# thebasilisk/mirror-maze

Measured on AMD Instinct MI355X. Metric: Mrays/sec + ms/frame at 1920x1080, 8 spp, 8 bounces; 1/2/4/8-GPU scaling, higher is better.
Workload: dtype f32

## Files before the change

### mirror-maze_amd/csrc/grid_build.cpp

```cpp
#include <algorithm>
#include <cmath>
#include <cstdint>
#include <cstring>
#include <string>
#include <vector>

#include "grid_build.h"
#include "mm_types.h"

namespace mm {

size_t build_compact_rects(const mm_rect* rects, uint32_t n_rects, const uint32_t* idx, std::vector<uint32_t>& out,
                           size_t* n_slow);

namespace {

void rect_box(const mm_rect& r, double lo[3], double hi[3]) {
    for (int a = 0; a < 3; ++a) {
        const double c[4] = {r.o[a], (double)r.o[a] + r.v[a], (double)r.o[a] + r.u[a],
                             (double)r.o[a] + r.v[a] + r.u[a]};
        lo[a] = *std::min_element(c, c + 4);
        hi[a] = *std::max_element(c, c + 4);
    }
}
// ... 251 lines not shown
    }
    g.n_list = (uint32_t)ext.size();
    g.off_list = align16(8u * (uint32_t)total);
    g.off_recs = align16(g.off_list + 2u * g.n_list);
    g.off_box = align16(g.off_recs + 32u * n_rects);
    g.bytes = align16(g.off_box + 24u * n_rects);
    g.image.assign(g.bytes, 0);
    std::memcpy(&g.image[0], words.data(), 8 * (size_t)total);
    if (!ext.empty()) std::memcpy(&g.image[g.off_list], ext.data(), 2 * ext.size());
    return true;
}

}

bool build_grid(const mm_rect* rects, uint32_t n_rects, const mm_node* nodes, uint32_t n_nodes,
                const uint32_t* idx, size_t index_budget, GridHost& g, std::string& why, bool merge_axes,
                double cell_scale, bool wide) {
    if (n_rects == 0 || n_rects > 65535) { why = "rect count outside 1..65535"; return false; }
    std::vector<uint32_t> ident(n_rects), recs;
    for (uint32_t k = 0; k < n_rects; ++k) ident[k] = k;
    size_t n_slow = 0;
    build_compact_rects(rects, n_rects, ident.data(), recs, &n_slow);
    double smin[3] = {INFINITY, INFINITY, INFINITY}, smax[3] = {-INFINITY, -INFINITY, -INFINITY}, C = 1.0;
    std::vector<double> ext2;
    for (uint32_t k = 0; k < n_rects; ++k) {
        double lo[3], hi[3];
        rect_box(rects[k], lo, hi);
        double e[3];
        for (int a = 0; a < 3; ++a) {
            if (!std::isfinite(lo[a]) || !std::isfinite(hi[a])) { why = "non-finite rect"; return false; }
            smin[a] = std::min(smin[a], lo[a]);
            smax[a] = std::max(smax[a], hi[a]);
            C = std::max(C, std::max(std::fabs(lo[a]), std::fabs(hi[a])));
            e[a] = hi[a] - lo[a];
        }
        std::sort(e, e + 3);
        if (e[1] > 0.0) ext2.push_back(e[1]);
    }
    if (ext2.empty()) { why = "no rect with area"; return false; }
    std::nth_element(ext2.begin(), ext2.begin() + ext2.size() / 2, ext2.end());
    std::vector<uint32_t> grecs;
    const uint32_t n_slow_g = grid_records(recs, n_rects, grecs);
    std::vector<uint32_t> cls;
    std::vector<uint32_t> cls_of(n_rects, 0);
    bool classes_ok = n_slow_g == 0;
    auto y_first = [&](uint32_t k) { return ((grecs[8 * (size_t)k + 7] >> 20) & 3u) == 2u; };
    for (uint32_t k = 0; k < n_rects && classes_ok; ++k) {
        const uint32_t* g8 = &grecs[8 * (size_t)k + 3];
        uint32_t t[4] = {g8[0], g8[1], g8[2], g8[3]};
        if (y_first(k)) { std::swap(t[0], t[2]); std::swap(t[1], t[3]); }
        uint32_t c = 0;
        while (c < cls.size() / 4 && !std::equal(t, t + 4, &cls[4 * c])) ++c;
        if (c == cls.size() / 4) {
            if (c == kMaxClasses) { classes_ok = false; break; }
            cls.insert(cls.end(), t, t + 4);
        }
        cls_of[k] = c;
    }
    auto maze_form = [&](const GridHost& gg) {
        if (gg.n[1] != 1 || !classes_ok || n_rects > 8191u) return false;
        for (uint32_t k = 0; k < n_rects; ++k) {
            const uint32_t meta = grecs[8 * (size_t)k + 7];
            const bool global = std::find(gg.glob, gg.glob + gg.n_glob, k) != gg.glob + gg.n_glob;
            if (!global && (meta >> 30) == 0u && ((meta >> 20) & 3u) == 1u) return false;
        }
        return true;
    };
    auto compact_layout = [&](GridHost& gg) {
        gg.off_class = gg.off_data = align16(gg.off_list + 2u * gg.n_list);
        gg.off_recs = gg.off_class + kGridClassBytes;
        gg.off_box = align16(gg.off_recs + 16u * n_rects);
        gg.bytes = align16(gg.off_box + 24u * n_rects);
    };
    double s = ext2[ext2.size() / 2] * cell_scale;
    for (int attempt = 0; attempt < 24; ++attempt, s *= 1.25) {
        if (wide && build_lists(rects, n_rects, recs, smin, smax, C, s, true, merge_axes, g, why)) {
            const bool mf = maze_form(g);
            if (mf) compact_layout(g);
            bool whole = false;
            for (size_t c = 0; mf && c < (size_t)g.n[0] * g.n[1] * g.n[2]; ++c)
                whole |= (g.image[8 * c + 7] & 0x80u) != 0;
            if (g.bytes <= index_budget && !whole) break;
        }
        if (build_lists(rects, n_rects, recs, smin, smax, C, s, false, merge_axes, g, why) &&
            g.off_recs <= index_budget)
            break;
        if (attempt == 23) { why = "no grid index fits the LDS budget"; return false; }
    }
    g.n_slow = n_slow_g;
    g.flat_ok = maze_form(g);
    if (g.wide && g.flat_ok) {
        for (size_t c = 0; c < (size_t)g.n[0] * g.n[1] * g.n[2]; ++c) {
            uint64_t w;
            std::memcpy(&w, &g.image[8 * c], 8);
            const uint64_t xf = (w >> 25) & 0xFFFull;
            w = (w & ~(0xFFFull << 37)) | (xf << 37);
            std::memcpy(&g.image[8 * c], &w, 8);
        }
    }
    g.slab = false;
    if (g.n_glob == 2) {
        const uint32_t m0 = grecs[8 * (size_t)g.glob[0] + 7], m1 = grecs[8 * (size_t)g.glob[1] + 7];
        const bool y_fast = (m0 >> 30) == 0u && (m1 >> 30) == 0u && ((m0 >> 20) & 3u) == 1u && ((m1 >> 20) & 3u) == 1u;
        float y0, y1;
        std::memcpy(&y0, &grecs[8 * (size_t)g.glob[0]], 4);
        std::memcpy(&y1, &grecs[8 * (size_t)g.glob[1]], 4);
        if (y_fast && y0 != y1 && std::isfinite(y0) && std::isfinite(y1)) {
            if (y1 < y0) { std::swap(g.glob[0], g.glob[1]); std::swap(y0, y1); }
            g.slab = true;
            g.slab_y[0] = y0;
            g.slab_y[1] = y1;
        }
    }
    if (g.flat_ok) {
        g.n_class = (uint32_t)cls.size() / 4;
        compact_layout(g);
        g.image.resize(g.bytes);
        std::memset(&g.image[g.off_recs], 0, g.bytes - g.off_recs);
        for (uint32_t k = 0; k < n_rects; ++k) {
            const uint32_t* w = &grecs[8 * (size_t)k];
            const uint32_t meta = (w[7] & (3u << 20)) | (cls_of[k] << 4) | (w[7] & (3u << 30));
            const uint32_t r[4] = {w[0], y_first(k) ? w[2] : w[1], y_first(k) ? w[1] : w[2], meta};
            std::memcpy(&g.image[g.off_recs + 16u * k], r, 16);
        }
        std::memcpy(&g.image[g.off_class], cls.data(), 4 * cls.size());
        for (uint32_t i = 0; i < g.n_list; ++i) {
            uint16_t e;
            std::memcpy(&e, &g.image[g.off_list + 2u * i], 2);
            e = (uint16_t)(8u * e);
            std::memcpy(&g.image[g.off_list + 2u * i], &e, 2);
        }
    } else {
        g.off_class = 0;
        g.off_data = g.off_recs;
        g.off_box = align16(g.off_recs + 32u * n_rects);
        g.bytes = align16(g.off_box + 24u * n_rects);
        g.image.resize(g.bytes);
        std::memcpy(&g.image[g.off_recs], grecs.data(), 32u * (size_t)n_rects);
    }
    std::vector<float> box(6 * (size_t)n_rects);
    for (uint32_t k = 0; k < n_rects; ++k) {
        const float e[6] = {INFINITY, -INFINITY, INFINITY, -INFINITY, INFINITY, -INFINITY};
        std::memcpy(&box[6 * (size_t)k], e, sizeof e);
    }
    for (uint32_t i = 0; i < n_nodes; ++i) {
        const mm_node& nd = nodes[i];
        if (nd.count == 0) continue;
        for (uint32_t j = 0; j < nd.count; ++j) {
            const uint32_t k = idx[nd.left_first + j];
            const float b[6] = {nd.mn[0], nd.mx[0], nd.mn[1], nd.mx[1], nd.mn[2], nd.mx[2]};
            std::memcpy(&box[6 * (size_t)k], b, sizeof b);
        }
    }
    std::memcpy(&g.image[g.off_box], box.data(), 24u * (size_t)n_rects);
    return true;
}

}
```

### mirror-maze_amd/csrc/grid_build.h

```cpp
#pragma once

#include <cstddef>
#include <cstdint>
#include <string>
#include <vector>

#include "mm_types.h"

namespace mm {

constexpr uint32_t kMaxClasses = 64;
constexpr uint32_t kGridClassBytes = 16 * kMaxClasses;

struct GridHost {
    float mn[3], mx[3], cell[3], inv[3];
    int n[3];
    uint32_t n_glob = 0;
    uint32_t glob[4] = {0, 0, 0, 0};
    uint32_t off_list = 0, off_recs = 0, off_box = 0, bytes = 0;
    uint32_t n_list = 0;
    uint32_t n_slow = 0;
    bool wide = true;
    bool flat_ok = false;
    bool slab = false;
    float slab_y[2] = {0.0f, 0.0f};
    uint32_t off_class = 0, n_class = 0;
    uint32_t off_data = 0;
    std::vector<uint8_t> image;
};

bool build_grid(const mm_rect* rects, uint32_t n_rects, const mm_node* nodes, uint32_t n_nodes,
                const uint32_t* idx, size_t index_budget, GridHost& g, std::string& why, bool merge_axes = true,
                double cell_scale = 1.0, bool wide = true);

}
```

### mirror-maze_amd/csrc/mm_device.h

```cpp
#pragma once

#include <hip/hip_runtime.h>
#include <stdint.h>

#include "grid_build.h"
#include "mm_types.h"
#include "mm_variants.h"

namespace mm {

constexpr float kBig = 1e30f;
constexpr int kStackMax = 50;

constexpr uint32_t kLaneStatRecord = 49152;
#ifdef MM_LANE_STATS
__device__ __forceinline__ uint32_t* lane_stat_words() {
    __shared__ uint32_t words[2 * kLpCount];
    return words;
}
__device__ __forceinline__ void lane_stat(int ph) {
    const uint64_t m = __ballot(1);
    if (__lane_id() == (uint32_t)(__ffsll((unsigned long long)m) - 1)) {
        atomicAdd(lane_stat_words() + 2 * ph, 1u);
        atomicAdd(lane_stat_words() + 2 * ph + 1, (uint32_t)__popcll(m));
    }
}
#define MM_LANE_STAT(ph) ::mm::lane_stat(::mm::ph)
#else
#define MM_LANE_STAT(ph) ((void)0)
#endif

__host__ __device__ constexpr bool grid_form(int f) { return f >= kFormGrid && f <= kFormGridWideSlow + kFormGridFlat; }
__host__ __device__ constexpr bool grid_flat(int f) { return f > kFormGridWideSlow; }
__host__ __device__ constexpr int grid_base(int f) { return grid_flat(f) ? f - kFormGridFlat : f; }
__host__ __device__ constexpr bool grid_slow(int f) { return grid_base(f) == kFormGridSlow || grid_base(f) == kFormGridWideSlow; }
__host__ __device__ constexpr bool grid_wide(int f) { return grid_base(f) >= kFormGridWide; }

struct DevGrid {
    float mn[3], mx[3];
    float cell[3], inv[3];
    int n[3];
    uint32_t n_glob;
    uint32_t glob[4];
    const void* cells;
    const uint16_t* list;
    const uint4* recs;
    const float2* box;
    const uint4* image;
    uint32_t off_list, off_recs, off_box, bytes;
    const float4* cls;
    uint32_t off_class;
    uint32_t off_data;
    uint32_t slab;
    float slab_y[2];
    int nm1[3];
    float nf[3];
};
inline DevGrid dev_grid(const GridHost& gh, const uint8_t* image_dev) {
    DevGrid dg{};
    for (int a = 0; a < 3; ++a) {
        dg.mn[a] = gh.mn[a]; dg.mx[a] = gh.mx[a]; dg.cell[a] = gh.cell[a]; dg.inv[a] = gh.inv[a];
        dg.n[a] = gh.n[a];
        dg.nm1[a] = gh.n[a] - 1;
        dg.nf[a] = (float)gh.n[a];
    }
    dg.n_glob = gh.n_glob;
    dg.slab = gh.slab ? 1u : 0u;
    dg.slab_y[0] = gh.slab_y[0];
    dg.slab_y[1] = gh.slab_y[1];
    for (int i = 0; i < 4; ++i) dg.glob[i] = gh.glob[i];
    dg.cells = image_dev;
    dg.list = reinterpret_cast<const uint16_t*>(image_dev + gh.off_list);
    dg.recs = reinterpret_cast<const uint4*>(image_dev + gh.off_recs);
    dg.box = reinterpret_cast<const float2*>(image_dev + gh.off_box);
    dg.image = reinterpret_cast<const uint4*>(image_dev);
    dg.off_list = gh.off_list; dg.off_recs = gh.off_recs; dg.off_box = gh.off_box; dg.bytes = gh.bytes;
    dg.off_class = gh.off_class;
    dg.off_data = gh.off_data;
    dg.cls = gh.off_class ? reinterpret_cast<const float4*>(image_dev + gh.off_class) : nullptr;
    return dg;
}

struct DevScene {
    const float4* nodes;
    const float4* nodes_ref;
    const float4* geo;
    const float4* shade;
    const uint32_t* idx;
    uint32_t n_nodes;
    uint32_t n_rects;
    uint32_t root_packed;
    uint32_t fast_ok;
    const uint2* recs;
    DevGrid grid;
};

struct F3 { float x, y, z; };
__device__ __forceinline__ F3 f3(float x, float y, float z) { return F3{x, y, z}; }
__device__ __forceinline__ F3 operator+(F3 a, F3 b) { return F3{a.x + b.x, a.y + b.y, a.z + b.z}; }
__device__ __forceinline__ F3 operator-(F3 a, F3 b) { return F3{a.x - b.x, a.y - b.y, a.z - b.z}; }
__device__ __forceinline__ F3 operator*(F3 a, F3 b) { return F3{a.x * b.x, a.y * b.y, a.z * b.z}; }
__device__ __forceinline__ F3 operator*(float s, F3 a) { return F3{s * a.x, s * a.y, s * a.z}; }
__device__ __forceinline__ float dot3(F3 a, F3 b) {
    float s = a.x * b.x;
    s = s + a.y * b.y;
    return s + a.z * b.z;
}
__device__ __forceinline__ float rsq_ieee(float x) { return 1.0f / sqrtf(x); }
__device__ __forceinline__ float rsq(float x) {
    if (x >= 0x1p-40f && x <= 0x1p40f) {
        float s = __builtin_amdgcn_sqrtf(x);
        const float sd = __uint_as_float(__float_as_uint(s) - 1u), su = __uint_as_float(__float_as_uint(s) + 1u);
        const float vd = __builtin_fmaf(-sd, s, x), vu = __builtin_fmaf(-su, s, x);
        s = vd <= 0.0f ? sd : s;
        s = vu > 0.0f ? su : s;
        const float y = __builtin_amdgcn_rcpf(s);
        const float e = __builtin_fmaf(-s, y, 1.0f);
        return __builtin_fmaf(e, y, y);
    }
    return rsq_ieee(x);
}
__device__ __forceinline__ F3 normalize3(F3 v) { return rsq(dot3(v, v)) * v; }
__device__ __forceinline__ F3 cross3(F3 v, F3 u) {
    return F3{u.z * v.y - u.y * v.z, u.x * v.z - u.z * v.x, u.y * v.x - u.x * v.y};
}
__device__ __forceinline__ F3 xyz(float4 a) { return F3{a.x, a.y, a.z}; }

__device__ __forceinline__ float rand_pm1(uint32_t& state) {
    uint32_t s = state * 747796405u + 291336453u;
    state = s;
    uint32_t r = ((s >> ((s >> 28) + 4u)) ^ s) * 277803737u;
    r = (r >> 22) ^ r;
    return __builtin_fmaf((float)r, 0x1p-31f, -1.0f);
}

__device__ __forceinline__ uint32_t cvt_u32_sat(float f) {
    if (!(f > 0.0f)) return 0u;
    if (f >= 4294967296.0f) return 0xFFFFFFFFu;
    return (uint32_t)f;
}

__device__ __forceinline__ uint32_t seed_reference(uint32_t tx, uint32_t ty, uint32_t time) {
    const float n = 128.0f / 255.0f;
    float s = n + (float)(tx * 15823u);
    s = s + n;
    s = s + (float)(ty * 9737333u);
    s = s + (float)time;
    return cvt_u32_sat(s);
}

__device__ __forceinline__ uint32_t pcg_hash(uint32_t v) {
    uint32_t s = v * 747796405u + 2891336453u;
    uint32_t w = ((s >> ((s >> 28) + 4u)) ^ s) * 277803737u;
    return (w >> 22) ^ w;
}
__device__ __forceinline__ uint32_t seed_tile(uint32_t pixel, uint32_t sample, uint32_t frame) {
    return pcg_hash(pcg_hash(pcg_hash(frame) ^ pixel) + sample);
}

__device__ __forceinline__ F3 primary_dir(const mm_uniform& u, uint32_t px, uint32_t py) {
    const float fx = (float)px, fy = (float)py;
    const float vx = u.cam.viewport[0], vy = u.cam.viewport[1];
    F3 p = F3{(vx * fx) / u.view_w - vx * 0.5f, (vy * fy) / u.view_h - vy * 0.5f, 0.0f - (-u.cam.focal)};
    F3 d = normalize3(p);
    const F3 q = F3{u.cam.quat[0], u.cam.quat[1], u.cam.quat[2]};
    const float qw = u.cam.quat[3];
    const F3 nq = F3{-q.x, -q.y, -q.z};
    const float s1 = -dot3(nq, d);
    const F3 c1 = F3{nq.y * d.z - nq.z * d.y, nq.z * d.x - nq.x * d.z, nq.x * d.y - nq.y * d.x};
    const F3 v1 = c1 + qw * d;
    const F3 c2 = F3{v1.y * q.z - v1.z * q.y, v1.z * q.x - v1.x * q.z, v1.x * q.y - v1.y * q.x};
    return (qw * v1 + s1 * q) + c2;
}

__device__ __forceinline__ F3 jitter(F3 d, uint32_t& seed) {
    const float j1 = rand_pm1(seed);
    const float j2 = rand_pm1(seed);
    return d + F3{j1 * 0.001f, j2 * 0.001f, 0.0f * 0.001f};
}

__device__ __forceinline__ float msign(float x) {
    if (x > 0.0f) return 1.0f;
    if (x < 0.0f) return -1.0f;
    if (x != x) return 0.0f;
    return x;
}

__device__ __forceinline__ uint32_t unorm8(float x) {
    x = fminf(fmaxf(x, 0.0f), 1.0f);
    return (uint32_t)rintf(x * 255.0f);
}

}
```

### mirror-maze_amd/csrc/mm_grid.h

```cpp
#pragma once

#include "mm_trace.h"

namespace mm {

__device__ __forceinline__ void grid_update(float a, uint32_t k, float& best, uint32_t& bk, uint32_t& tie) {
    if (a < best) {
        best = a;
        bk = k;
        tie = 0u;
    } else if (a == best && k != bk) {
        tie = 1u;
    }
}

__device__ __forceinline__ void grid_update_sel(float a, uint32_t k, float& best, uint32_t& bk, uint32_t& tie) {
    const bool lt = a < best, eq = (a == best) & (k != bk);
    tie = lt ? 0u : (tie | (eq ? 1u : 0u));
    bk = lt ? k : bk;
    best = lt ? a : best;
}

__device__ __forceinline__ void grid_rect_general(const float4* __restrict__ geo, uint32_t k, uint32_t e,
                                                  const Ray& r, float& best, uint32_t& bk, uint32_t& tie) {
// ... 202 lines not shown
                                            const Ray& r, float& t, uint32_t& index, Counters& c) {
    float best = kBig;
    uint32_t bk = 0xFFFFFFFFu;
    uint32_t tie = 0u;
    bool one = false;
    uint32_t k1 = 0;
    if (arg_at_use(g.slab)) {
        const float q = 0.05f * r.d.y;
        const bool lo_dead = r.d.y > 0.0f && g.slab_y[0] - r.o.y <= q;
        const bool hi_dead = r.d.y < 0.0f && g.slab_y[1] - r.o.y >= q;
        one = __builtin_amdgcn_ballot_w64(!(lo_dead || hi_dead)) == 0;
        k1 = rect_name<kFlat>(lo_dead ? g.glob[1] : g.glob[0]);
    }
    if (one) {
        MM_LANE_STAT(kLpGlobal);
        grid_rect_axis<1, kFlat>(gv, k1, rec_words<kFlat>(gv, k1), r, best, bk, tie);
    } else {
        for (uint32_t j = 0, n = arg_at_use(g.n_glob); j < n; ++j) {
            MM_LANE_STAT(kLpGlobal);
            grid_rect_uniform<kSlow, kFlat>(gv, geo, rect_name<kFlat>(g.glob[j]), r, best, bk, tie);
        }
    }
    const float s0 = 0.09375f;
    int bx = grid_first(g, 0, r.o.x + s0 * r.d.x, r.y.x),
        by = kFlat ? (r.y.y > 0.0f ? 1 : 0) : grid_first(g, 1, r.o.y + s0 * r.d.y, r.y.y),
        bz = grid_first(g, 2, r.o.z + s0 * r.d.z, r.y.z);
    const float Ax = (g.mn[0] - r.o.x) * r.y.x, Bx = g.cell[0] * r.y.x;
    const float Az = (g.mn[2] - r.o.z) * r.y.z, Bz = g.cell[2] * r.y.z;
    const float Ay = kFlat ? 0.0f : (g.mn[1] - r.o.y) * r.y.y, By = kFlat ? 0.0f : g.cell[1] * r.y.y;
    float tx = __builtin_fmaf((float)bx, Bx, Ax), tz = __builtin_fmaf((float)bz, Bz, Az);
    float ty = kFlat ? grid_time(g, 1, by, r.o.y, r.y.y) : __builtin_fmaf((float)by, By, Ay);
    int ci;
    {
        const int ix = r.y.x > 0.0f ? bx - 1 : bx, iz = r.y.z > 0.0f ? bz - 1 : bz;
        const int iy = kFlat ? 0 : (r.y.y > 0.0f ? by - 1 : by);
        ci = kFlat ? iz * g.n[0] + ix : (iz * g.n[1] + iy) * g.n[0] + ix;
    }
    constexpr int kCs = decltype(gv.cells)::template kScale<kWide>;
    uint32_t cp = gv.cells.template pos<kWide>(ci);
    const int dcx = r.y.x > 0.0f ? kCs : -kCs;
    const int dcz = (r.y.z > 0.0f ? kCs : -kCs) * (kFlat ? g.n[0] : g.n[0] * g.n[1]);
    const int dcy = kFlat ? 0 : (r.y.y > 0.0f ? kCs : -kCs) * g.n[0];
    const uint32_t fsh = (25u + (r.y.x > 0.0f ? 0u : 6u)) | ((37u + (r.y.y > 0.0f ? 0u : 6u)) << 8) |
                         ((49u + (r.y.z > 0.0f ? 0u : 6u)) << 16);
    uint32_t j, jend;
    auto cell_pos = [&](uint32_t sh) {
        constexpr bool kB = decltype(gv.list)::kStep == 2u;
        if constexpr (kWide && kFlat) {
            const uint64_t cw = gv.cells.at64(cp);
            const uint32_t lo = (uint32_t)cw, first = lo & 0x3FFFFFu;
            if (sh == 0u) {
                j = first;
                jend = first + (kB ? (lo >> 21) & 0xEu : (lo >> 22) & 7u);
            } else {
                const uint32_t f = (uint32_t)(cw >> 32) >> sh;
                j = first + (kB ? (twice(f) & 14u) : (f & 7u));
                jend = j + (kB ? ((f >> 2) & 14u) : ((f >> 3) & 7u));
            }
        } else if constexpr (kWide) {
            const uint64_t cw = gv.cells.at64(cp);
            const uint32_t lo = (uint32_t)cw;
            const bool whole = (int32_t)(uint32_t)(cw >> 32) < 0;
            const uint32_t first = lo & 0x3FFFFFu;
            const uint32_t m = kB ? (lo >> 21) & (whole ? 0x7FEu : 0xEu) : (lo >> 22) & (whole ? 0x3FFu : 7u);
            if (sh == 0u) {
                j = first;
                jend = first + m;
            } else {
                const uint32_t f = (uint32_t)(cw >> sh);
                const uint32_t st = kB ? (twice(f) & 14u) : (f & 7u), len = kB ? ((f >> 2) & 14u) : ((f >> 3) & 7u);
                j = first + (whole ? 0u : st);
                jend = j + (whole ? m : len);
            }
        } else {
            const uint32_t cw = gv.cells.at32(cp);
            j = cw & 0x3FFFFFu;
            jend = j + (kB ? ((cw >> 21) & 0x7FEu) : (cw >> 22));
        }
    };
    cell_pos(0u);
    uint32_t cells = 1, tests = g.n_glob;
    if constexpr (kFlat) {
        const float sgx = r.y.x > 0.0f ? 1.0f : -1.0f, sgz = r.y.z > 0.0f ? 1.0f : -1.0f;
        float fbx = (float)bx, fbz = (float)bz;
        const float tend = fminf(ty, fminf(__builtin_fmaf(r.y.x > 0.0f ? g.nf[0] : 0.0f, Bx, Ax),
                                           __builtin_fmaf(r.y.z > 0.0f ? g.nf[2] : 0.0f, Bz, Az)));
        const uint32_t shx = kWide ? (r.y.x > 0.0f ? 5u : 11u) : 0u, shz = kWide ? (r.y.z > 0.0f ? 17u : 23u) : 0u;
        for (;;) {
            MM_LANE_STAT(kLpGridIter);
            if (j < jend) {
                do {
                    MM_LANE_STAT(kLpRectTest);
                    grid_rect<kSlow, kFlat, kFlat>(gv, geo, gv.list.at(j), r, best, bk, tie);
                    j += gv.list.kStep;
                    if (kStats) ++tests;
                } while (j < jend);
            }
            MM_LANE_STAT(kLpCellStep);
            const bool sx = tx <= tz;
            const float te = sx ? tx : tz;
            if (!(te <= best) | !(te < tend)) break;
            fbx = sx ? fbx + sgx : fbx;
            fbz = sx ? fbz : fbz + sgz;
            tx = sx ? __builtin_fmaf(fbx, Bx, Ax) : tx;
            tz = sx ? tz : __builtin_fmaf(fbz, Bz, Az);
            cp += (uint32_t)(sx ? dcx : dcz);
            cell_pos(sx ? shx : shz);
            if (kStats) ++cells;
        }
    } else {
        for (;;) {
            MM_LANE_STAT(kLpGridIter);
            if (j < jend) {
                do {
                    MM_LANE_STAT(kLpRectTest);
                    grid_rect<kSlow, kFlat, kFlat>(gv, geo, gv.list.at(j), r, best, bk, tie);
                    j += gv.list.kStep;
                    if (kStats) ++tests;
                } while (j < jend);
            }
            {
                MM_LANE_STAT(kLpCellStep);
                const float te = fminf(tx, fminf(ty, tz));
                if (best < te) break;
                const bool sx = tx == te, sy = !sx && ty == te, sz = !sx && !sy;
                bx += sx ? (r.y.x > 0.0f ? 1 : -1) : 0;
                by += sy ? (r.y.y > 0.0f ? 1 : -1) : 0;
                bz += sz ? (r.y.z > 0.0f ? 1 : -1) : 0;
                if (((uint32_t)bx > (uint32_t)g.n[0]) | ((uint32_t)by > (uint32_t)g.n[1]) |
                    ((uint32_t)bz > (uint32_t)g.n[2]))
                    break;
                const int b = sx ? bx : (sy ? by : bz);
                const float nt = __builtin_fmaf((float)b, sel_xy(sx, sy, F3{Bx, By, Bz}),
                                                sel_xy(sx, sy, F3{Ax, Ay, Az}));
                tx = sx ? nt : tx;
                ty = sy ? nt : ty;
                tz = sz ? nt : tz;
                cp += (uint32_t)(sx ? dcx : (sy ? dcy : dcz));
                cell_pos((fsh >> (sx ? 0u : (sy ? 8u : 16u))) & 0xFFu);
                if (kStats) ++cells;
            }
        }
    }
    if (kStats) {
        c.visits += cells;
        c.rtests += tests;
    }
    if (best == kBig) {
        t = kBig;
        return !tie;
    }
    if (tie) return false;
    MM_LANE_STAT(kLpCert);
    const float2* bp = kFlat ? reinterpret_cast<const float2*>(reinterpret_cast<const char*>(gv.box) + (bk + twice(bk)))
                             : gv.box + 3 * bk;
    bk = rect_index<kFlat>(bk);
    const float2 bxx = bp[0], byy = bp[1], bzz = bp[2];
    const float tx1 = qdiv(bxx.x - r.o.x, r.d.x, r.y.x), tx2 = qdiv(bxx.y - r.o.x, r.d.x, r.y.x);
    float tmin = fminf(tx1, tx2), tmax = fmaxf(tx1, tx2);
    const float ty1 = qdiv(byy.x - r.o.y, r.d.y, r.y.y), ty2 = qdiv(byy.y - r.o.y, r.d.y, r.y.y);
    tmin = fmaxf(tmin, fminf(ty1, ty2));
    tmax = fminf(tmax, fmaxf(ty1, ty2));
    const float tz1 = qdiv(bzz.x - r.o.z, r.d.z, r.y.z), tz2 = qdiv(bzz.y - r.o.z, r.d.z, r.y.z);
    tmin = fmaxf(tmin, fminf(tz1, tz2));
    tmax = fminf(tmax, fmaxf(tz1, tz2));
    if (!(tmax >= tmin && tmax > 0.0f && tmin <= best)) return false;
    t = best;
    index = bk;
    return true;
}

}
```

### mirror-maze_amd/csrc/mm_runtime.hip

```cpp
#include <hip/hip_runtime.h>

#include <algorithm>
#include <chrono>
#include <cmath>
#include <cstdio>
#include <cstring>
#include <deque>
#include <new>
#include <string>
#include <thread>
#include <vector>

#include "grid_build.h"
#include "mm_aov.h"
#include "mm_api.h"
#include "mm_ctx.h"
#include "mm_launch.h"
#include "mm_plan.h"

using namespace mm;

namespace mm {
size_t build_compact_rects(const mm_rect* rects, uint32_t n_rects, const uint32_t* idx, std::vector<uint32_t>& out,
                           size_t* n_slow);
// ... 350 lines not shown
            if (value != -1 && value != 0 && value != 5 && value != 7 && value != 11)
                return fail(c, MM_ERR_INVALID, "traversal must be -1 (auto), 0, 5, 7 or 11 (grid search)");
            if (value == 0) return fail(c, MM_ERR_UNSUPPORTED, kRemoved);
            c->opt_ww = value;
            return MM_OK;
        case MM_OPT_LDS_RECTS: c->opt_lds_rects = value != 0; return MM_OK;
        case MM_OPT_LDS_SPLIT:
            if (value < 0) return fail(c, MM_ERR_INVALID, "split cache size must be >= 0 (0 off, 1 auto, else KB)");
            if (value > 1) return fail(c, MM_ERR_UNSUPPORTED, kRemoved);
            return MM_OK;
        case MM_OPT_FUSE_RESOLVE: c->opt_fuse = value != 0; return MM_OK;
        case MM_OPT_RESERVE_CUS:
            if (value < 0 || value > 128) return fail(c, MM_ERR_INVALID, "reserved CUs must be 0..128");
            c->opt_reserve_cus = (uint32_t)value;
            return MM_OK;
        case MM_OPT_DEFER:
            if (value < 0 || value > 64) return fail(c, MM_ERR_INVALID, "defer lanes must be 0..64");
            c->opt_defer = value;
            return MM_OK;
        case MM_OPT_DEFER_MIN:
            if (value < 0) return fail(c, MM_ERR_INVALID, "defer min paths must be >= 0");
            c->opt_defer_min = (uint32_t)value;
            return MM_OK;
        case MM_OPT_DICT_NODES:
            if (value < 0 || value > 2) return fail(c, MM_ERR_INVALID, "dict nodes must be 0, 1 or 2");
            if (value == 2) return fail(c, MM_ERR_UNSUPPORTED, kRemoved);
            return MM_OK;
        case MM_OPT_GRID_MERGE: c->opt_grid_merge = value != 0; return MM_OK;
        case MM_OPT_GRID_WIDE: c->opt_grid_wide = value != 0; return MM_OK;
        case MM_OPT_GRID_CELL:
            if (value < 25 || value > 400) return fail(c, MM_ERR_INVALID, "grid cell scale must be 25..400 (%)");
            c->opt_grid_cell = value;
            return MM_OK;
        case MM_OPT_FAULT_INJECT:
            if (value < 0 || value > 4) return fail(c, MM_ERR_INVALID, "fault inject must be 0..4");
            c->opt_fault = value;
            return MM_OK;
        default: return fail(c, MM_ERR_INVALID, "unknown option");
    }
}

int mm_scene_info(const mm_ctx* c, int key, double* value) {
    if (!c || !value) return MM_ERR_INVALID;
    if (!c->has_scene) return MM_ERR_NO_SCENE;
    const DevGrid& g = c->grid;
    switch (key) {
        case MM_INFO_GRID_OK: *value = c->grid_ok ? 1.0 : 0.0; return MM_OK;
        case MM_INFO_GRID_CELLS_X: *value = g.n[0]; return MM_OK;
        case MM_INFO_GRID_CELLS_Y: *value = g.n[1]; return MM_OK;
        case MM_INFO_GRID_CELLS_Z: *value = g.n[2]; return MM_OK;
        case MM_INFO_GRID_GLOBAL: *value = g.n_glob; return MM_OK;
        case MM_INFO_GRID_BYTES: *value = g.bytes; return MM_OK;
        case MM_INFO_GRID_INDEX_BYTES: *value = g.off_data; return MM_OK;
        case MM_INFO_LEAN: *value = c->lean_ok ? 1.0 : 0.0; return MM_OK;
        case MM_INFO_DEPTH: *value = c->depth; return MM_OK;
        case MM_INFO_DICT_OK: *value = 0.0; return MM_OK;
        case MM_INFO_LAST_FORM: *value = c->last_form; return MM_OK;
        case MM_INFO_LAST_LDS_MODE: *value = c->last_mode; return MM_OK;
        case MM_INFO_GRID_FACES: *value = c->grid_ok && c->grid_wide ? 1.0 : 0.0; return MM_OK;
        case MM_INFO_LAST_DEFER: *value = c->last_defer ? 1.0 : 0.0; return MM_OK;
        case MM_INFO_GRID_LDS_CAP: *value = wavepersist_grid_cap(0); return MM_OK;
        case MM_INFO_GRID_FLAT: *value = c->grid_ok && c->grid_flat ? 1.0 : 0.0; return MM_OK;
        case MM_INFO_GRID_SLAB: *value = c->grid_ok && g.slab && g.slab_y[0] < g.slab_y[1] ? 1.0 : 0.0; return MM_OK;
        case MM_INFO_GRID_CLASSES: *value = c->grid_ok ? c->grid_classes : 0u; return MM_OK;
        case MM_INFO_LAST_VGPRS:
        case MM_INFO_LAST_SCRATCH:
        case MM_INFO_LAST_STATIC_LDS: {
            if (c->last_kern_mode < 0) return MM_ERR_INVALID;
            hipFuncAttributes a{};
            if (wavepersist_attributes(c->last_kern_mode, c->last_kern_form, c->last_kern_ring, &a) != hipSuccess)
                return MM_ERR_HIP;
            *value = key == MM_INFO_LAST_VGPRS ? a.numRegs
                     : key == MM_INFO_LAST_SCRATCH ? (double)a.localSizeBytes : (double)a.sharedSizeBytes;
            return MM_OK;
        }
        default: return MM_ERR_INVALID;
    }
}

int mm_upload_scene(mm_ctx* c, const mm_rect* rects, uint32_t n_rects, const mm_node* nodes, uint32_t n_nodes,
                    const uint32_t* idx, const uint8_t* is_mirror, const float* emission) {
    if (!c) return MM_ERR_INVALID;
    if (!rects || !nodes || !idx || !is_mirror || !emission || n_rects == 0 || n_nodes == 0)
        return fail(c, MM_ERR_INVALID, "mm_upload_scene: null array or empty scene");
    if (n_nodes > 2 * n_rects) return fail(c, MM_ERR_INVALID, "mm_upload_scene: more than 2n-1 nodes");
    std::string why;
    uint32_t depth = 0;
    int rc = check_tree(nodes, n_nodes, idx, n_rects, why, &depth);
    if (rc != MM_OK) return fail(c, rc, "mm_upload_scene: " + why);
    for (uint32_t i = 0; i < n_nodes; ++i)
        if (nodes[i].count >= 256u || nodes[i].left_first >= (1u << 24))
            return fail(c, MM_ERR_UNSUPPORTED, "mm_upload_scene: leaf with >= 256 planes or index >= 2^24");
    std::vector<uint32_t> pair_old;
    if (nodes[0].count == 0) pair_old.push_back(nodes[0].left_first);
    for (size_t q = 0; q < pair_old.size(); ++q)
        for (uint32_t k = 0; k < 2; ++k) {
            const mm_node& nd = nodes[pair_old[q] + k];
            if (nd.count == 0) pair_old.push_back(nd.left_first);
        }
    std::vector<uint32_t> pair_new(n_nodes, 0);
    for (size_t q = 0; q < pair_old.size(); ++q) pair_new[pair_old[q]] = 2 + 2 * (uint32_t)q;
    if (2 + 2 * pair_old.size() >= (1u << 24))
        return fail(c, MM_ERR_UNSUPPORTED, "mm_upload_scene: node index >= 2^24");
    auto pack = [&](const mm_node& nd) {
        return nd.count > 0 ? (nd.count << 24) | nd.left_first : pair_new[nd.left_first];
    };
    const uint32_t n_prod = 2 + 2 * (uint32_t)pair_old.size();
    std::vector<float4> packed(2 * (size_t)n_prod, make_float4(0.0f, 0.0f, 0.0f, 0.0f));
    for (size_t q = 0; q < pair_old.size(); ++q)
        for (uint32_t k = 0; k < 2; ++k) {
            const mm_node& nd = nodes[pair_old[q] + k];
            const uint32_t pk = pack(nd);
            float pkf;
            std::memcpy(&pkf, &pk, 4);
            const size_t i = 2 + 2 * q + k;
            packed[2 * i] = make_float4(nd.mn[0], nd.mx[0], nd.mn[1], nd.mx[1]);
            packed[2 * i + 1] = make_float4(nd.mn[2], nd.mx[2], pkf, 0.0f);
        }
    bool fast = true;
    for (uint32_t i = 0; i < n_nodes && fast; ++i)
        for (int a = 0; a < 3; ++a) fast = fast && coord_ok(nodes[i].mn[a]) && coord_ok(nodes[i].mx[a]);
    for (uint32_t k = 0; k < n_rects && fast; ++k)
        for (int a = 0; a < 3; ++a)
            fast = fast && coord_ok(rects[k].o[a]) && extent_ok(rects[k].v[a]) && extent_ok(rects[k].u[a]);
    HIPC(c, hipSetDevice(c->device));
    free_scene(c);
    std::vector<float4> shade(2 * (size_t)n_rects);
    for (uint32_t k = 0; k < n_rects; ++k) {
        shade[2 * k] = make_float4(rects[k].color[0], rects[k].color[1], rects[k].color[2], is_mirror[k] ? 1.0f : 0.0f);
        shade[2 * k + 1] = make_float4(emission[4 * k], emission[4 * k + 1], emission[4 * k + 2], emission[4 * k + 3]);
    }
    HIPC(c, hipMalloc((void**)&c->d_rects, n_rects * sizeof(mm_rect)));
    HIPC(c, hipMalloc((void**)&c->d_nodes, packed.size() * sizeof(float4)));
    HIPC(c, hipMalloc((void**)&c->d_nodes_ref, n_nodes * sizeof(mm_node)));
    HIPC(c, hipMalloc((void**)&c->d_geo, 4 * (size_t)n_rects * sizeof(float4)));
    HIPC(c, hipMalloc((void**)&c->d_shade, 2 * (size_t)n_rects * sizeof(float4)));
    HIPC(c, hipMalloc((void**)&c->d_idx, n_rects * sizeof(uint32_t)));
    std::vector<uint32_t> recs;
    size_t n_slow = n_rects;
    c->n_fast_recs = n_rects < (1u << 20) ? build_compact_rects(rects, n_rects, idx, recs, &n_slow) : 0;
    if (n_rects >= (1u << 20)) recs.assign(10 * (size_t)n_rects, 2u << 30);
    HIPC(c, hipMalloc((void**)&c->d_recs, recs.size() * sizeof(uint32_t)));
    HIPC(c, hipMemcpyAsync(c->d_recs, recs.data(), recs.size() * sizeof(uint32_t), hipMemcpyHostToDevice, c->stream));
    HIPC(c, hipMemcpyAsync(c->d_rects, rects, n_rects * sizeof(mm_rect), hipMemcpyHostToDevice, c->stream));
    HIPC(c, hipMemcpyAsync(c->d_nodes_ref, nodes, n_nodes * sizeof(mm_node), hipMemcpyHostToDevice, c->stream));
    HIPC(c, hipMemcpyAsync(c->d_nodes, packed.data(), packed.size() * sizeof(float4), hipMemcpyHostToDevice, c->stream));
    GridHost gh;
    std::string gwhy;
    const bool grid_ok = fast && build_grid(rects, n_rects, nodes, n_nodes, idx, wavepersist_grid_cap(0), gh, gwhy,
                                            c->opt_grid_merge, c->opt_grid_cell / 100.0, c->opt_grid_wide);
    if (!fast) gwhy = "scene coordinates outside the exact-division guards";
    DevGrid dg{};
    if (grid_ok) {
        HIPC(c, hipMalloc((void**)&c->d_grid, gh.bytes));
        HIPC(c, hipMemcpyAsync(c->d_grid, gh.image.data(), gh.bytes, hipMemcpyHostToDevice, c->stream));
        dg = dev_grid(gh, c->d_grid);
        c->grid_slow = gh.n_slow > 0;
        c->grid_wide = gh.wide;
        c->grid_flat = gh.flat_ok;
        c->grid_classes = gh.n_class;
    }
    HIPC(c, hipMemcpyAsync(c->d_shade, shade.data(), shade.size() * sizeof(float4), hipMemcpyHostToDevice, c->stream));
    HIPC(c, hipMemcpyAsync(c->d_idx, idx, n_rects * sizeof(uint32_t), hipMemcpyHostToDevice, c->stream));
    HIPC(c, launch_prep_rects(c->d_rects, n_rects, c->d_geo, c->stream));
    HIPC(c, hipStreamSynchronize(c->stream));
    c->n_rects = n_rects;
    c->n_nodes = n_prod;
    c->root_packed = pack(nodes[0]);
    c->depth = depth;
    c->fast_ok = fast;
    c->lean_ok = n_slow == 0;
    c->grid = dg;
    c->grid_ok = grid_ok;
    c->grid_why = grid_ok ? std::string() : gwhy;
    c->has_scene = true;
    return MM_OK;
}

int mm_trace_chunks(mm_ctx* c, const mm_uniform* u, const uint32_t* chunks, uint32_t n_chunks) {
    if (!c) return MM_ERR_INVALID;
    if (!c->has_scene) return fail(c, MM_ERR_NO_SCENE, "mm_trace_chunks: no scene uploaded");
    if (!u || !chunks) return fail(c, MM_ERR_INVALID, "mm_trace_chunks: null argument");
    if (!(u->view_w >= 1.0f && u->view_w <= 65536.0f && u->view_h >= 1.0f && u->view_h <= 65536.0f))
        return fail(c, MM_ERR_INVALID, "mm_trace_chunks: bad view size");
    if (u->chunk_w != 4) return fail(c, MM_ERR_UNSUPPORTED, "mm_trace_chunks: chunk_w must be 4 (64 samples/pixel)");
    const uint32_t ppc = 16;
    const uint32_t gw = (uint32_t)(u->view_w / 2.0f / (float)ppc), gh = (uint32_t)(u->view_h / 2.0f / (float)ppc);
    if (gw == 0 || gh == 0) return fail(c, MM_ERR_INVALID, "mm_trace_chunks: view too small for one group");
    uint32_t max_pbi = 0;
    for (uint32_t gy = 0; gy < gh; ++gy) {
        float f = ((u->view_w * 0.5f) * (float)gy) / (float)ppc + (float)(gw - 1);
        max_pbi = std::max(max_pbi, (uint32_t)f);
    }
    if (max_pbi >= n_chunks) return fail(c, MM_ERR_INVALID, "mm_trace_chunks: chunk list shorter than the grid");
    const uint32_t W = (uint32_t)u->view_w, H = (uint32_t)u->view_h;
    HIPC(c, hipSetDevice(c->device));
    if (W != c->fb_w || H != c->fb_h) {
        (void)hipFree(c->d_fb); (void)hipFree(c->d_fb8); (void)hipFree(c->d_fb8_alt);
        c->d_fb = nullptr; c->d_fb8 = nullptr; c->d_fb8_alt = nullptr;
        c->fb_w = c->fb_h = 0;
        HIPC(c, hipMalloc((void**)&c->d_fb, (size_t)W * H * sizeof(float4)));
        HIPC(c, hipMalloc((void**)&c->d_fb8, (size_t)W * H * sizeof(uint32_t)));
        HIPC(c, hipMalloc((void**)&c->d_fb8_alt, (size_t)W * H * sizeof(uint32_t)));
        HIPC(c, hipMemsetAsync(c->d_fb, 0, (size_t)W * H * sizeof(float4), c->stream));
        HIPC(c, hipMemsetAsync(c->d_fb8, 0, (size_t)W * H * sizeof(uint32_t), c->stream));
        c->fb_w = W; c->fb_h = H;
    }
    int rc = ensure(c, c->d_chunks, c->chunks_cap, 2 * (size_t)n_chunks);
    if (rc) return rc;
    HIPC(c, hipMemcpyAsync(c->d_chunks, chunks, 2 * (size_t)n_chunks * sizeof(uint32_t), hipMemcpyHostToDevice,
                           c->stream));
    HIPC(c, hipMemsetAsync(c->d_aux, 0, 5 * sizeof(unsigned long long), c->stream));
    if ((rc = begin_timing(c))) return rc;
    HIPC(c, launch_trace_chunks(dev_scene(c), *u, c->d_chunks, gw, gh, c->d_fb, c->d_fb8, c->d_aux,
                                reinterpret_cast<uint32_t*>(c->d_aux + 4), false, c->stream));
    if ((rc = end_timing(c, 1))) return rc;
    c->last_chunks = n_chunks;
    return read_aux(c, nullptr);
}

int mm_present(mm_ctx* c) {
    if (!c) return MM_ERR_INVALID;
    if (!c->d_fb8) return fail(c, MM_ERR_INVALID, "mm_present: nothing rendered yet");
    HIPC(c, hipSetDevice(c->device));
    HIPC(c, launch_present_blur(c->d_fb8, c->d_fb8_alt, c->fb_w, c->fb_h, c->stream));
    std::swap(c->d_fb8, c->d_fb8_alt);
    return MM_OK;
}

int mm_read_packets(mm_ctx* c, float* packets, uint32_t n_chunks) {
    if (!c) return MM_ERR_INVALID;
    if (!packets) return fail(c, MM_ERR_INVALID, "mm_read_packets: null output");
    if (!c->d_fb || c->last_chunks == 0) return fail(c, MM_ERR_INVALID, "mm_read_packets: no mm_trace_chunks yet");
    if (n_chunks > c->last_chunks)
        return fail(c, MM_ERR_INVALID, "mm_read_packets: more chunks than the last dispatch used");
    if (n_chunks == 0) return MM_OK;
    HIPC(c, hipSetDevice(c->device));
    int rc = ensure(c, c->d_packets, c->packets_cap, 16 * (size_t)n_chunks);
    if (rc) return rc;
    HIPC(c, launch_chunk_packets(c->d_fb, c->d_chunks, n_chunks, c->fb_w, c->fb_h, c->d_packets, c->stream));
    HIPC(c, hipMemcpyAsync(packets, c->d_packets, 16 * (size_t)n_chunks * sizeof(float4), hipMemcpyDeviceToHost,
                           c->stream));
    HIPC(c, hipStreamSynchronize(c->stream));
    return MM_OK;
}

int mm_quantize_rgba8(mm_ctx* c, const float* rgba_dev, uint8_t* rgba8_dev, uint64_t n_pixels) {
    if (!c) return MM_ERR_INVALID;
    if ((!rgba_dev || !rgba8_dev) && n_pixels) return fail(c, MM_ERR_INVALID, "mm_quantize_rgba8: null buffer");
    if (n_pixels == 0) return MM_OK;
    if (reinterpret_cast<uintptr_t>(rgba_dev) % 16 || reinterpret_cast<uintptr_t>(rgba8_dev) % 4)
        return fail(c, MM_ERR_INVALID, "mm_quantize_rgba8: misaligned buffer");
    HIPC(c, hipSetDevice(c->device));
    HIPC(c, launch_quantize(reinterpret_cast<const float4*>(rgba_dev), reinterpret_cast<uint32_t*>(rgba8_dev),
                            (size_t)n_pixels, c->stream));
    return MM_OK;
}

int mm_denoise_frames(mm_ctx* c, const float* color_dev, const mm_aov* guides, const mm_denoise_params* p,
                      uint32_t n_frames, uint32_t w, uint32_t h, void* out_dev) {
    if (!p || !guides || !color_dev || !out_dev) return fail(c, MM_ERR_INVALID, "mm_denoise_frames: null argument");
    if (!guides->normal_depth || !guides->albedo || !guides->id)
        return fail(c, MM_ERR_INVALID, "mm_denoise_frames: all three guide buffers are required");
    if (p->n_passes < 1 || p->n_passes > MM_DENOISE_MAX_PASSES)
        return fail(c, MM_ERR_INVALID, "mm_denoise_frames: n_passes must be 1..8");
    if (p->flags & ~MM_DN_RGBA8) return fail(c, MM_ERR_INVALID, "mm_denoise_frames: unknown flags");
    if (w == 0 || h == 0 || n_frames == 0) return fail(c, MM_ERR_INVALID, "mm_denoise_frames: empty tile or no frames");
    const bool rgba8 = (p->flags & MM_DN_RGBA8) != 0;
    if (reinterpret_cast<uintptr_t>(color_dev) % 16 || reinterpret_cast<uintptr_t>(guides->normal_depth) % 16 ||
        reinterpret_cast<uintptr_t>(guides->albedo) % 16 || reinterpret_cast<uintptr_t>(guides->id) % 4 ||
        reinterpret_cast<uintptr_t>(out_dev) % (rgba8 ? 4 : 16))
        return fail(c, MM_ERR_INVALID, "mm_denoise_frames: misaligned buffer (float4: 16 bytes, id and RGBA8: 4)");
    const uint64_t n_pix = (uint64_t)w * h;
    if (n_pix > 0x7FFFFFFFull || n_pix * n_frames > (1ull << 40))
        return fail(c, MM_ERR_INVALID, "mm_denoise_frames: more pixels than one call holds");
    const uint64_t n_all = n_pix * n_frames, out_bytes = n_all * (rgba8 ? 4 : 16);
    if (ranges_overlap(out_dev, out_bytes, color_dev, n_all * 16) ||
        ranges_overlap(out_dev, out_bytes, guides->normal_depth, n_all * 16) ||
        ranges_overlap(out_dev, out_bytes, guides->albedo, n_all * 16) ||
        ranges_overlap(out_dev, out_bytes, guides->id, n_all * 4))
        return fail(c, MM_ERR_INVALID, "mm_denoise_frames: the output overlaps an input");
    if (!c) return MM_ERR_INVALID;
    HIPC(c, hipSetDevice(c->device));
    const uint32_t n_passes = p->n_passes;
    if (n_passes > 1)
        if (int rc = dn_scratch(c, c->d_dn_img, c->dn_img_cap, (n_passes > 2 ? 2 : 1) * (size_t)n_pix)) return rc;
    if (int rc = dn_scratch(c, c->d_dn_keys, c->dn_keys_cap, (size_t)n_all)) return rc;
    if (!c->dn_done) HIPC(c, hipEventCreateWithFlags(&c->dn_done, hipEventDisableTiming));
    if (c->dn_pending && c->dn_stream != c->stream) HIPC(c, hipStreamWaitEvent(c->stream, c->dn_done, 0));
    const float4* color = reinterpret_cast<const float4*>(color_dev);
    HIPC(c, launch_denoise_keys(reinterpret_cast<const float4*>(guides->albedo), guides->id, c->d_dn_keys,
                                (size_t)n_all, c->stream));
    c->dn_pending = true;
    c->dn_stream = c->stream;
    for (uint32_t f = 0; f < n_frames; ++f) {
        const size_t o = (size_t)f * n_pix;
        DnPass a;
        a.nd = reinterpret_cast<const float4*>(guides->normal_depth) + o;
        a.keys = c->d_dn_keys + o;
        a.w = w; a.h = h;
        a.sigma_z = p->sigma_z; a.sigma_l = p->sigma_l;
        a.in = color + o;
        for (uint32_t i = 0; i < n_passes; ++i) {
            const bool last = i + 1 == n_passes;
            a.s = 1u << i;
            a.sl = p->sigma_l * (1.0f / (float)a.s);
            a.rgba8 = last && rgba8;
            if (last) a.out = rgba8 ? (void*)(reinterpret_cast<uint8_t*>(out_dev) + o * 4)
// ... 324 lines not shown
```

### mirror-maze_amd/csrc/mm_variants.h

```cpp
#pragma once

#include <cstddef>
#include <cstdint>

namespace mm {

enum LanePhase : int {
    kLpChunk, kLpBounce, kLpGlobal, kLpGridIter, kLpRectTest, kLpCellStep, kLpCert, kLpFallback,
    kLpShade, kLpDiffuse, kLpTrial, kLpMirror, kLpCount
};

enum : int {
    kFormIfIf = 0, kFormLeafInterior = 5, kFormLean = 7,
    kFormGrid = 11, kFormGridSlow = 12, kFormGridWide = 13, kFormGridWideSlow = 14,
    kFormGridFlat = 4
};

enum LdsMode : int {
    kLdsNone = 0,
    kLdsNodes = 1,
    kLdsNodesRecs = 3,
    kLdsGridImage = 11,
    kLdsGridIndex = 12,
    kLdsGridNone = 13,
    kLdsGridData = 14,
};
constexpr bool lds_static_grid(int mode) { return mode == kLdsGridImage || mode == kLdsGridData; }
constexpr bool lds_whole_search(int mode) { return mode == kLdsGridImage || mode == kLdsNodesRecs; }

constexpr size_t lds_stage_bytes(int mode, uint32_t n_nodes, uint32_t n_rects, uint32_t grid_bytes,
                                 uint32_t grid_off_data, uint32_t grid_off_box) {
    switch (mode) {
        case kLdsGridImage: return grid_bytes;
        case kLdsGridIndex: return grid_off_data;
        case kLdsGridData: return grid_off_box;
        case kLdsNodes: return 32 * (size_t)n_nodes;
        case kLdsNodesRecs: return 32 * (size_t)n_nodes + 40 * (size_t)n_rects;
        default: return 0;
    }
}

constexpr uint32_t kLdsPerBlock = 80 * 1024;

constexpr uint32_t kTailRing = 512;
#ifdef MM_TAIL_CLOCKS
constexpr uint32_t kClaimWords = 16;
#else
constexpr uint32_t kClaimWords = 2;
#endif

template <int kRing>
constexpr uint32_t grid_lds_cap() {
    uint32_t other = kClaimWords * 16u * 4u + 64u;
    if (kRing != 0) other += (4u + kTailRing) * 4u;
    if (kRing == 2) other += 4u * kTailRing * 16u;
#ifdef MM_LANE_STATS
    other += 2u * kLpCount * 4u;
#endif
    return (kLdsPerBlock - other) & ~15u;
}
constexpr uint32_t wavepersist_grid_cap(int ring) {
    return ring == 2 ? grid_lds_cap<2>() : ring == 1 ? grid_lds_cap<1>() : grid_lds_cap<0>();
}

#define MM_FLAT_INSTANCES(X)                                                                                  \
    X(11, kFormGridWide + kFormGridFlat) X(11, kFormGrid + kFormGridFlat) X(14, kFormGrid + kFormGridFlat)     \
    X(12, kFormGrid + kFormGridFlat) X(13, kFormGridWide + kFormGridFlat) X(13, kFormGrid + kFormGridFlat)
#define MM_DEFER_INSTANCES(X)                                                                                 \
    X(11, kFormGrid) X(12, kFormGrid) X(13, kFormGrid)                                                        \
    X(11, kFormGridSlow) X(12, kFormGridSlow) X(13, kFormGridSlow)                                            \
    X(11, kFormGridWide) X(13, kFormGridWide) X(11, kFormGridWideSlow) X(13, kFormGridWideSlow)               \
    MM_FLAT_INSTANCES(X) X(3, kFormLean)
#define MM_PLAIN_INSTANCES(X) X(0, kFormLeafInterior) X(1, kFormLeafInterior) X(3, kFormLeafInterior)
#define MM_WP_INSTANCES(X) MM_DEFER_INSTANCES(X) MM_PLAIN_INSTANCES(X)

constexpr bool wavepersist_defer_built(int lds_mode, int form) {
#define MM_WP(L, F) if (lds_mode == (L) && form == (F)) return true;
    MM_DEFER_INSTANCES(MM_WP)
    return false;
}
constexpr bool wavepersist_built(int lds_mode, int form) {
    if (wavepersist_defer_built(lds_mode, form)) return true;
    MM_PLAIN_INSTANCES(MM_WP)
#undef MM_WP
    return false;
}

enum AovPolicy : int {
    kAovRef = 0,
    kAovBvhLi = 1,
    kAovBvhLean = 2,
    kAovGrid = 3,
    kAovGridSlow = 1, kAovGridWide = 2, kAovGridFlat = 4,
};
#define MM_AOV_POLICIES(X)                                                                                   \
    X(kAovRef) X(kAovBvhLi) X(kAovBvhLean) X(kAovGrid) X(kAovGrid + kAovGridSlow) X(kAovGrid + kAovGridWide) \
    X(kAovGrid + kAovGridWide + kAovGridSlow) X(kAovGrid + kAovGridFlat) X(kAovGrid + kAovGridFlat + kAovGridWide)
constexpr bool aov_policy_built(int policy) {
#define MM_AOV(P) if (policy == (P)) return true;
    MM_AOV_POLICIES(MM_AOV)
#undef MM_AOV
    return false;
}

}
```

Measured before the change: 68740.

## Replace per-hit slab box certification with precomputed point-in-window check

The hit certification step used to run a full slab test (six guarded divisions) against the leaf box for every candidate hit. It now stores a per-rect conservative window (center and half-width, shrunk by a margin) in the staged box slot and first checks whether the hit point lies inside it with a few FMAs and compares. Only rays that fail this cheap test load the original boxes, now held in a separate buffer after the grid image, and run the full slab test. This adds an extra device allocation, host precompute and a divergent fallback path, and correctness depends on the window margins being conservative.

```diff
diff --git a/mirror-maze_amd/csrc/grid_build.cpp b/mirror-maze_amd/csrc/grid_build.cpp
--- a/mirror-maze_amd/csrc/grid_build.cpp
+++ b/mirror-maze_amd/csrc/grid_build.cpp
@@ -427,7 +427,33 @@
             std::memcpy(&box[6 * (size_t)k], b, sizeof b);
         }
     }
-    std::memcpy(&g.image[g.off_box], box.data(), 24u * (size_t)n_rects);
+    g.win_m = (float)std::ldexp(C, -20);
+    g.omax = (float)(8.0 * C);
+    std::vector<float> win(6 * (size_t)n_rects);
+    for (uint32_t k = 0; k < n_rects; ++k) {
+        const float* b = &box[6 * (size_t)k];
+        float* w = &win[6 * (size_t)k];
+        const uint32_t meta = grecs[8 * (size_t)k + 7], ak = (meta >> 20) & 3u;
+        float ok;
+        std::memcpy(&ok, &grecs[8 * (size_t)k], 4);
+        const bool covered = (meta >> 30) == 0u && ak < 3u && b[2 * ak] <= ok && ok <= b[2 * ak + 1];
+        for (uint32_t a = 0; a < 3; ++a) {
+            float c = 0.0f, h = -1.0f;
+            if (covered && a == ak) {
+                h = INFINITY;
+            } else if (covered) {
+                const double xl = (double)b[2 * a] + (double)g.win_m, xh = (double)b[2 * a + 1] - (double)g.win_m;
+                c = (float)(0.5 * (xl + xh));
+                const double hd = std::min((double)c - xl, xh - (double)c) * (1.0 - 0x1p-22);
+                h = (float)hd;
+                if ((double)h > hd) h = std::nextafterf(h, -INFINITY);
+            }
+            w[2 * a] = c;
+            w[2 * a + 1] = h;
+        }
+    }
+    std::memcpy(&g.image[g.off_box], win.data(), 24u * (size_t)n_rects);
+    g.boxes = std::move(box);
     return true;
 }
 
diff --git a/mirror-maze_amd/csrc/grid_build.h b/mirror-maze_amd/csrc/grid_build.h
--- a/mirror-maze_amd/csrc/grid_build.h
+++ b/mirror-maze_amd/csrc/grid_build.h
@@ -26,6 +26,9 @@
     float slab_y[2] = {0.0f, 0.0f};
     uint32_t off_class = 0, n_class = 0;
     uint32_t off_data = 0;
+    float win_m = 0.0f;
+    float omax = 0.0f;
+    std::vector<float> boxes;
     std::vector<uint8_t> image;
 };
 
diff --git a/mirror-maze_amd/csrc/mm_device.h b/mirror-maze_amd/csrc/mm_device.h
--- a/mirror-maze_amd/csrc/mm_device.h
+++ b/mirror-maze_amd/csrc/mm_device.h
@@ -46,6 +46,8 @@
     const uint16_t* list;
     const uint4* recs;
     const float2* box;
+    const float2* cbox;
+    float omax;
     const uint4* image;
     uint32_t off_list, off_recs, off_box, bytes;
     const float4* cls;
@@ -73,6 +75,8 @@
     dg.list = reinterpret_cast<const uint16_t*>(image_dev + gh.off_list);
     dg.recs = reinterpret_cast<const uint4*>(image_dev + gh.off_recs);
     dg.box = reinterpret_cast<const float2*>(image_dev + gh.off_box);
+    dg.cbox = reinterpret_cast<const float2*>(image_dev + gh.bytes);
+    dg.omax = gh.omax;
     dg.image = reinterpret_cast<const uint4*>(image_dev);
     dg.off_list = gh.off_list; dg.off_recs = gh.off_recs; dg.off_box = gh.off_box; dg.bytes = gh.bytes;
     dg.off_class = gh.off_class;
diff --git a/mirror-maze_amd/csrc/mm_grid.h b/mirror-maze_amd/csrc/mm_grid.h
--- a/mirror-maze_amd/csrc/mm_grid.h
+++ b/mirror-maze_amd/csrc/mm_grid.h
@@ -378,19 +378,30 @@
     }
     if (tie) return false;
     MM_LANE_STAT(kLpCert);
-    const float2* bp = kFlat ? reinterpret_cast<const float2*>(reinterpret_cast<const char*>(gv.box) + (bk + twice(bk)))
+    const float2* wp = kFlat ? reinterpret_cast<const float2*>(reinterpret_cast<const char*>(gv.box) + (bk + twice(bk)))
                              : gv.box + 3 * bk;
     bk = rect_index<kFlat>(bk);
-    const float2 bxx = bp[0], byy = bp[1], bzz = bp[2];
-    const float tx1 = qdiv(bxx.x - r.o.x, r.d.x, r.y.x), tx2 = qdiv(bxx.y - r.o.x, r.d.x, r.y.x);
-    float tmin = fminf(tx1, tx2), tmax = fmaxf(tx1, tx2);
-    const float ty1 = qdiv(byy.x - r.o.y, r.d.y, r.y.y), ty2 = qdiv(byy.y - r.o.y, r.d.y, r.y.y);
-    tmin = fmaxf(tmin, fminf(ty1, ty2));
-    tmax = fminf(tmax, fmaxf(ty1, ty2));
-    const float tz1 = qdiv(bzz.x - r.o.z, r.d.z, r.y.z), tz2 = qdiv(bzz.y - r.o.z, r.d.z, r.y.z);
-    tmin = fmaxf(tmin, fminf(tz1, tz2));
-    tmax = fminf(tmax, fmaxf(tz1, tz2));
-    if (!(tmax >= tmin && tmax > 0.0f && tmin <= best)) return false;
+    const float2 wx = wp[0], wy = wp[1], wz = wp[2];
+    const float px = __builtin_fmaf(best, r.d.x, r.o.x), py = __builtin_fmaf(best, r.d.y, r.o.y),
+                pz = __builtin_fmaf(best, r.d.z, r.o.z);
+    bool clear = fmaxf(fmaxf(fabsf(r.o.x), fabsf(r.o.y)), fabsf(r.o.z)) <= g.omax;
+    clear &= fabsf(px - wx.x) <= wx.y;
+    clear &= fabsf(py - wy.x) <= wy.y;
+    clear &= fabsf(pz - wz.x) <= wz.y;
+    if (!clear) {
+        MM_LANE_STAT(kLpCertFull);
+        const float2* bp = g.cbox + 3 * bk;
+        const float2 bxx = bp[0], byy = bp[1], bzz = bp[2];
+        const float tx1 = qdiv(bxx.x - r.o.x, r.d.x, r.y.x), tx2 = qdiv(bxx.y - r.o.x, r.d.x, r.y.x);
+        float tmin = fminf(tx1, tx2), tmax = fmaxf(tx1, tx2);
+        const float ty1 = qdiv(byy.x - r.o.y, r.d.y, r.y.y), ty2 = qdiv(byy.y - r.o.y, r.d.y, r.y.y);
+        tmin = fmaxf(tmin, fminf(ty1, ty2));
+        tmax = fminf(tmax, fmaxf(ty1, ty2));
+        const float tz1 = qdiv(bzz.x - r.o.z, r.d.z, r.y.z), tz2 = qdiv(bzz.y - r.o.z, r.d.z, r.y.z);
+        tmin = fmaxf(tmin, fminf(tz1, tz2));
+        tmax = fminf(tmax, fmaxf(tz1, tz2));
+        if (!(tmax >= tmin && tmax > 0.0f && tmin <= best)) return false;
+    }
     t = best;
     index = bk;
     return true;
diff --git a/mirror-maze_amd/csrc/mm_runtime.hip b/mirror-maze_amd/csrc/mm_runtime.hip
--- a/mirror-maze_amd/csrc/mm_runtime.hip
+++ b/mirror-maze_amd/csrc/mm_runtime.hip
@@ -526,8 +526,10 @@
     if (!fast) gwhy = "scene coordinates outside the exact-division guards";
     DevGrid dg{};
     if (grid_ok) {
-        HIPC(c, hipMalloc((void**)&c->d_grid, gh.bytes));
+        const size_t box_bytes = gh.boxes.size() * sizeof(float);
+        HIPC(c, hipMalloc((void**)&c->d_grid, gh.bytes + box_bytes));
         HIPC(c, hipMemcpyAsync(c->d_grid, gh.image.data(), gh.bytes, hipMemcpyHostToDevice, c->stream));
+        HIPC(c, hipMemcpyAsync(c->d_grid + gh.bytes, gh.boxes.data(), box_bytes, hipMemcpyHostToDevice, c->stream));
         dg = dev_grid(gh, c->d_grid);
         c->grid_slow = gh.n_slow > 0;
         c->grid_wide = gh.wide;
diff --git a/mirror-maze_amd/csrc/mm_variants.h b/mirror-maze_amd/csrc/mm_variants.h
--- a/mirror-maze_amd/csrc/mm_variants.h
+++ b/mirror-maze_amd/csrc/mm_variants.h
@@ -7,7 +7,7 @@
 
 enum LanePhase : int {
     kLpChunk, kLpBounce, kLpGlobal, kLpGridIter, kLpRectTest, kLpCellStep, kLpCert, kLpFallback,
-    kLpShade, kLpDiffuse, kLpTrial, kLpMirror, kLpCount
+    kLpShade, kLpDiffuse, kLpTrial, kLpMirror, kLpCertFull, kLpCount
 };
 
 enum : int {
```

Measured after the change: 70060, median of 6. +1.9%, better.
